# BoMingZhao/GaussianPrediction

Measured on AMD Instinct MI355X. Metric: rendered views/s (full train step) @1M Gaussians 1352x1014, higher is better.
Workload: dtype f32; 1 GPU; configs[2]: HyperNeRF-like 1M Gaussians, 1352x1014, stage-3 full train step (deform, raster, L1+SSIM loss, Adam: all HIP kernels); gaussians=1000000, width=1352, height=1014, keypoints=250, nearest_num=6, parallelism=view-parallel x1, ranks_seen_by_rccl=1, self_launched=False

## Files before the change

### gaussianprediction_amd/csrc/deform_kernels.hip

```cpp
#include "gp_common.h"
#include "deform_kernels.h"

typedef float f32x16 __attribute__((ext_vector_type(16)));

#define MLP_ROWS 32
#define MLP_THREADS 512
#define MLP_W 256

__device__ __forceinline__ int act_idx(int f, int j) { return f * MLP_ROWS + (j ^ (f & 31)); }
__device__ __forceinline__ int cd_row(int r, int half) { return (r & 3) + 8 * (r >> 2) + 4 * half; }

__device__ __forceinline__ void build_input(float* buf, const MlpDev& p, long row0, int tid) {
    const int fd = p.feature_dim, xf = p.xyz_freq, tf = p.time_freq;
    for (int e = tid; e < fd * MLP_ROWS; e += MLP_THREADS) {
        const int jj = e / fd, f = e - jj * fd;
        const long row = row0 + jj;
        buf[act_idx(f, jj)] = row < p.rows ? p.feature[row * fd + f] : 0.f;
    }
    for (int e = tid; e < 3 * xf * MLP_ROWS; e += MLP_THREADS) {
        const int jj = e % MLP_ROWS, cf = e / MLP_ROWS;
        const int c = cf / xf, fr = cf - c * xf;
        const long row = row0 + jj;
        float sv = 0.f, cv = 0.f;
        if (row < p.rows) {
// ... 685 lines not shown
}
__global__ __launch_bounds__(256) void gp_blend_fwd_kernel(BlendDev a, float* __restrict__ xyz_t, float* __restrict__ q_t) { blend_fwd_body<0>(a, xyz_t, q_t); }
__global__ __launch_bounds__(256) void gp_blend_fwd6_kernel(BlendDev a, float* __restrict__ xyz_t, float* __restrict__ q_t) { blend_fwd_body<6>(a, xyz_t, q_t); }
__global__ __launch_bounds__(256) void gp_blend_fwd8_kernel(BlendDev a, float* __restrict__ xyz_t, float* __restrict__ q_t) { blend_fwd_body<8>(a, xyz_t, q_t); }
__global__ __launch_bounds__(256) void gp_blend_fwd6_i16_kernel(BlendDev a, float* __restrict__ xyz_t, float* __restrict__ q_t) { blend_fwd_body<6, true>(a, xyz_t, q_t); }
__global__ __launch_bounds__(256) void gp_blend_fwd8_i16_kernel(BlendDev a, float* __restrict__ xyz_t, float* __restrict__ q_t) { blend_fwd_body<8, true>(a, xyz_t, q_t); }

__device__ __forceinline__ void normalize_bwd(const float* v, const float* g, float* dv) {
    const float n = norm4(v), inv = 1.f / n;
    const float y[4] = {v[0] * inv, v[1] * inv, v[2] * inv, v[3] * inv};
    const float dot = y[0] * g[0] + y[1] * g[1] + y[2] * g[2] + y[3] * g[3];
#pragma unroll
    for (int k = 0; k < 4; ++k) dv[k] = (g[k] - y[k] * dot) * inv;
}

#define BB_LONG 20
#define BB_LONG_CAP 320
template <int NN, bool I16 = false>
__device__ __forceinline__ void blend_bwd_body(BlendDev a, const float* __restrict__ g_xyz_t,
                                               const float* __restrict__ g_q_t, float* __restrict__ g_delta,
                                               float* __restrict__ g_raw_w, float* __restrict__ g_xyz,
                                               float* __restrict__ g_rot, float* __restrict__ partial, const unsigned bid,
                                               const unsigned nblk) {
    extern __shared__ float s_dyn[];
    const int od = a.out_dim;
    const int nn = NN > 0 ? NN : a.nn;
    const int K = (int)a.K;
    const int tid = threadIdx.x;
    float* s_acc = s_dyn;
    float* s_delta = s_acc + (nn > 0 ? K * 7 : 0);
    int* s_cnt = (int*)(s_delta + (nn > 0 ? K * od : 0));
    int* s_base = s_cnt + (nn > 0 ? K : 0);
    float* s_g = (float*)(s_base + (nn > 0 ? K + 1 : 0));
    float* s_inv = s_g + 256 * 7;
    float* s_w = s_inv + (nn > 0 ? K : 0);
    unsigned short* s_sorted = (unsigned short*)(s_w + 256 * 2 * nn);
    __shared__ int s_wsum[4];
    __shared__ int s_nlong, s_long[BB_LONG_CAP];
    if (nn > 0) {
        for (int e = tid; e < K * 7; e += 256) s_acc[e] = 0.f;
        for (int e = tid; e < K * od; e += 256) s_delta[e] = a.delta[e];
        if (a.norm_rotation) {
            __syncthreads();
            for (int kp = tid; kp < K; kp += 256) {
                float* dl = s_delta + kp * od;
                const float v[4] = {dl[3], dl[4], dl[5], dl[6]};
                const float inv = 1.f / norm4(v);
                s_inv[kp] = inv;
                dl[3] = v[0] * inv; dl[4] = v[1] * inv; dl[5] = v[2] * inv; dl[6] = v[3] * inv;
            }
        }
    }
    const long chunks = (a.N + 255) / 256;
    for (long c = bid; c < chunks; c += nblk) {
        const long i = c * 256 + tid;
        const bool live = i < a.N;
        if (nn > 0) {
            for (int e = tid; e < K; e += 256) s_cnt[e] = 0;
            if (tid == 0) s_nlong = 0;
            __syncthreads();
        }
        int kps[NN > 0 ? NN : GP_MAX_NN], rk[NN > 0 ? NN : GP_MAX_NN];
        if (live) {
            const float gx[3] = {g_xyz_t[3 * i], g_xyz_t[3 * i + 1], g_xyz_t[3 * i + 2]};
            const float gq[4] = {g_q_t[4 * i], g_q_t[4 * i + 1], g_q_t[4 * i + 2], g_q_t[4 * i + 3]};
            const float r[4] = {a.rot[4 * i], a.rot[4 * i + 1], a.rot[4 * i + 2], a.rot[4 * i + 3]};
            float wx[NN > 0 ? NN : GP_MAX_NN], wr[NN > 0 ? NN : GP_MAX_NN];
            float dq[4] = {0.f, 0.f, 0.f, 0.f};
            if (nn > 0) {
                if constexpr (NN > 0) {
                    float raw[2 * (NN > 0 ? NN : 1)];
                    load_row_nn<NN, I16>(a, i, raw, kps);
                    softmax_n(raw, NN, wx);
                    softmax_n(raw + NN, NN, wr);
                } else {
                    softmax_n(a.raw_w + i * 2 * nn, nn, wx);
                    softmax_n(a.raw_w + i * 2 * nn + nn, nn, wr);
                }
#pragma unroll
                for (int k = 0; k < nn; ++k) {
                    if (NN == 0) kps[k] = a.knn16 ? (int)a.knn16[i * nn + k] : (int)a.knn[i * nn + k];
                    const float* dl = s_delta + kps[k] * od;
                    const float v[4] = {dl[3], dl[4], dl[5], dl[6]};
                    dq[0] = fmaf(wr[k], v[0], dq[0]); dq[1] = fmaf(wr[k], v[1], dq[1]);
                    dq[2] = fmaf(wr[k], v[2], dq[2]); dq[3] = fmaf(wr[k], v[3], dq[3]);
                }
            } else {
                const float* dl = a.delta + i * od;
                dq[0] = dl[3]; dq[1] = dl[4]; dq[2] = dl[5]; dq[3] = dl[6];
                if (a.norm_rotation) { const float inv = 1.f / norm4(dq); dq[0] *= inv; dq[1] *= inv; dq[2] *= inv; dq[3] *= inv; }
            }
            const float invq = 1.f / norm4(dq);
            const float q[4] = {dq[0] * invq, dq[1] * invq, dq[2] * invq, dq[3] * invq};
            g_xyz[3 * i] = gx[0]; g_xyz[3 * i + 1] = gx[1]; g_xyz[3 * i + 2] = gx[2];
            float pq[4];
            quat_mul(q, r, pq);
            float gp[4];
            normalize_bwd(pq, gq, gp);
            const float gqn[4] = {gp[0] * r[0] + gp[1] * r[1] + gp[2] * r[2] + gp[3] * r[3],
                                  -gp[0] * r[1] + gp[1] * r[0] - gp[2] * r[3] + gp[3] * r[2],
                                  -gp[0] * r[2] + gp[1] * r[3] + gp[2] * r[0] - gp[3] * r[1],
                                  -gp[0] * r[3] - gp[1] * r[2] + gp[2] * r[1] + gp[3] * r[0]};
            g_rot[4 * i + 0] = gp[0] * q[0] + gp[1] * q[1] + gp[2] * q[2] + gp[3] * q[3];
            g_rot[4 * i + 1] = -gp[0] * q[1] + gp[1] * q[0] + gp[2] * q[3] - gp[3] * q[2];
            g_rot[4 * i + 2] = -gp[0] * q[2] - gp[1] * q[3] + gp[2] * q[0] + gp[3] * q[1];
            g_rot[4 * i + 3] = -gp[0] * q[3] + gp[1] * q[2] - gp[2] * q[1] + gp[3] * q[0];
            float gdq[4];
            normalize_bwd(dq, gqn, gdq);
            if (nn > 0) {
                float gwx[NN > 0 ? NN : GP_MAX_NN], gwr[NN > 0 ? NN : GP_MAX_NN];
                float sx = 0.f, sr = 0.f;
#pragma unroll
                for (int k = 0; k < nn; ++k) {
                    const float* dl = s_delta + kps[k] * od;
                    gwx[k] = dl[0] * gx[0] + dl[1] * gx[1] + dl[2] * gx[2];
                    const float vn[4] = {dl[3], dl[4], dl[5], dl[6]};
                    gwr[k] = vn[0] * gdq[0] + vn[1] * gdq[1] + vn[2] * gdq[2] + vn[3] * gdq[3];
                    sx += wx[k] * gwx[k];
                    sr += wr[k] * gwr[k];
                    s_w[k * 256 + tid] = wx[k];
                    s_w[(nn + k) * 256 + tid] = wr[k];
// ... 16 lines not shown
                }
                s_g[0 * 256 + tid] = gx[0]; s_g[1 * 256 + tid] = gx[1]; s_g[2 * 256 + tid] = gx[2];
                s_g[3 * 256 + tid] = gdq[0]; s_g[4 * 256 + tid] = gdq[1]; s_g[5 * 256 + tid] = gdq[2]; s_g[6 * 256 + tid] = gdq[3];
            } else {
                const float* dl = a.delta + i * od;
                float gv[4] = {gdq[0], gdq[1], gdq[2], gdq[3]};
                if (a.norm_rotation) { const float v[4] = {dl[3], dl[4], dl[5], dl[6]}; normalize_bwd(v, gdq, gv); }
                float* gd = g_delta + i * od;
                gd[0] = gx[0]; gd[1] = gx[1]; gd[2] = gx[2];
                gd[3] = gv[0]; gd[4] = gv[1]; gd[5] = gv[2]; gd[6] = gv[3];
                for (int k = 7; k < od; ++k) gd[k] = 0.f;
            }
        }
        if (nn > 0) {
            __syncthreads();
            {
                const int per = (K + 255) / 256;
                const int b0 = tid * per;
                int loc = 0;
                for (int e = 0; e < per; ++e) if (b0 + e < K) loc += s_cnt[b0 + e];
                int inc = loc;
                inc = gp_wave_scan_add(inc);
                if ((tid & 63) == 63) s_wsum[tid >> 6] = inc;
                __syncthreads();
                int woff = 0;
                for (int w = 0; w < (tid >> 6); ++w) woff += s_wsum[w];
                int run = woff + inc - loc;
                for (int e = 0; e < per; ++e) if (b0 + e < K) { s_base[b0 + e] = run; run += s_cnt[b0 + e]; }
                if (tid == 255) s_base[K] = run;
            }
            __syncthreads();
            if (live) {
#pragma unroll
                for (int k = 0; k < nn; ++k) s_sorted[s_base[kps[k]] + rk[k]] = (unsigned short)((k << 8) | tid);
            }
            __syncthreads();
            for (int kp = tid; kp < K; kp += 256) {
                float sacc[7] = {0.f, 0.f, 0.f, 0.f, 0.f, 0.f, 0.f};
                const int pe = s_base[kp + 1];
                if (pe - s_base[kp] > BB_LONG) { s_long[atomicAdd(&s_nlong, 1)] = kp; continue; }
                for (int pp = s_base[kp]; pp < pe; pp += 2) {
                    const int e0 = s_sorted[pp], e1 = pp + 1 < pe ? s_sorted[pp + 1] : -1;
                    const int t0 = e0 & 255, k0 = e0 >> 8, t1 = e1 & 255, k1 = (e1 >> 8) & 15;
                    const float wx0 = s_w[k0 * 256 + t0], wr0 = s_w[(nn + k0) * 256 + t0];
                    const float wx1 = e1 >= 0 ? s_w[k1 * 256 + t1] : 0.f, wr1 = e1 >= 0 ? s_w[(nn + k1) * 256 + t1] : 0.f;
                    float g0[7], g1[7];
#pragma unroll
                    for (int cc = 0; cc < 7; ++cc) { g0[cc] = s_g[cc * 256 + t0]; g1[cc] = s_g[cc * 256 + t1]; }
                    sacc[0] = fmaf(wx0, g0[0], sacc[0]); sacc[1] = fmaf(wx0, g0[1], sacc[1]); sacc[2] = fmaf(wx0, g0[2], sacc[2]);
                    sacc[3] = fmaf(wr0, g0[3], sacc[3]); sacc[4] = fmaf(wr0, g0[4], sacc[4]);
                    sacc[5] = fmaf(wr0, g0[5], sacc[5]); sacc[6] = fmaf(wr0, g0[6], sacc[6]);
// ... 60 lines not shown
__global__ __launch_bounds__(256) void gp_blend_bwd8_i16_kernel(BB_ARGS) { blend_bwd_body<8, true>(a, g_xyz_t, g_q_t, g_delta, g_raw_w, g_xyz, g_rot, partial, blockIdx.x, gridDim.x); }

template <int NN, bool I16>
__device__ __forceinline__ void blend_bwd_ride_body(const BlendRideDev& r, BB_ARGS) {
    const unsigned riders = r.fin_blocks + r.adam_chunks;
    if (blockIdx.x < riders) {
        if (blockIdx.x < r.fin_blocks) {
            extern __shared__ float s_dyn[];
            double* s_tot = (double*)(((uintptr_t)s_dyn + 7) & ~(uintptr_t)7);
            loss_finalize_body(r.fin, (float*)(s_tot + 8), s_tot);
        } else {
            adam_chunk_body<256>(r.t, blockIdx.x - r.fin_blocks, threadIdx.x, r.b1, r.b2, r.eps, r.zero_grad, r.skip_flag);
        }
        return;
    }
    blend_bwd_body<NN, I16>(a, g_xyz_t, g_q_t, g_delta, g_raw_w, g_xyz, g_rot, partial, blockIdx.x - riders, gridDim.x - riders);
}
__global__ __launch_bounds__(256) void gp_blend_bwd6_ride_kernel(BlendRideDev r, BB_ARGS) { blend_bwd_ride_body<6, false>(r, a, g_xyz_t, g_q_t, g_delta, g_raw_w, g_xyz, g_rot, partial); }
__global__ __launch_bounds__(256) void gp_blend_bwd8_ride_kernel(BlendRideDev r, BB_ARGS) { blend_bwd_ride_body<8, false>(r, a, g_xyz_t, g_q_t, g_delta, g_raw_w, g_xyz, g_rot, partial); }
__global__ __launch_bounds__(256) void gp_blend_bwd6_i16_ride_kernel(BlendRideDev r, BB_ARGS) { blend_bwd_ride_body<6, true>(r, a, g_xyz_t, g_q_t, g_delta, g_raw_w, g_xyz, g_rot, partial); }
__global__ __launch_bounds__(256) void gp_blend_bwd8_i16_ride_kernel(BlendRideDev r, BB_ARGS) { blend_bwd_ride_body<8, true>(r, a, g_xyz_t, g_q_t, g_delta, g_raw_w, g_xyz, g_rot, partial); }

__global__ __launch_bounds__(1024) void gp_blend_bwd_reduce_kernel(const float* __restrict__ partial, int nblocks, int KA,
                                                                  int od, float* __restrict__ g_delta) {
    __shared__ float s_r[16][64];
    const int lane = threadIdx.x & 63, wave = threadIdx.x >> 6;
    const int e = blockIdx.x * 64 + lane;
    float v0 = 0.f, v1 = 0.f, v2 = 0.f, v3 = 0.f;
    if (e < KA) {
        int b = wave;
        for (; b + 240 < nblocks; b += 256) {
// ... 68 lines not shown
```

### gaussianprediction_amd/csrc/gp_capi_deform.hip

```cpp
#include "gp_common.h"
#include "deform_kernels.h"
#include "loss_adam_kernels.h"
#include <stdlib.h>

static int make_mlp(const gp_mlp_params* p, const gp_mlp_input* x, MlpDev& m) {
    if (!p || !x) GP_FAIL("null mlp params/input");
    if (p->width != 256 || p->depth != 4) GP_FAIL("Deformable_Field: only d=4, w=256 is implemented (got d=%d w=%d)", p->depth, p->width);
    if (p->out_dim < 7 || p->out_dim > 8) GP_FAIL("out_dim must be 7 or 8 (got %d)", p->out_dim);
    if (x->feature_dim <= 0 || x->feature_dim % 4 || x->xyz_freq < 0 || x->xyz_freq > 16 || x->time_freq < 0 || x->time_freq > 16)
        GP_FAIL("bad input encoding dims");
    const int in_dim = x->feature_dim + 6 * x->xyz_freq + 2 * x->time_freq;
    if (in_dim != p->in_dim) GP_FAIL("in_dim %d != feature_dim + 6*xyz_freq + 2*time_freq = %d", p->in_dim, in_dim);
    if (in_dim % 4 || in_dim > 256) GP_FAIL("in_dim %d must be a multiple of 4 and <= 256", in_dim);
    if (x->rows < 0) GP_FAIL("negative rows");
    for (int l = 0; l < 5; ++l)
        if (!p->w[l] || !p->b[l]) GP_FAIL("null weight pointer (layer %d)", l);
    if (x->rows > 0 && (!x->feature || (x->xyz_freq > 0 && !x->xyz) || (x->time_freq > 0 && !x->t))) GP_FAIL("null input pointer");
    m.rows = x->rows; m.in_dim = in_dim; m.in_pad = (in_dim + 7) / 8 * 8; m.out_dim = p->out_dim;
    m.feature_dim = x->feature_dim; m.xyz_freq = x->xyz_freq; m.time_freq = x->time_freq;
    for (int l = 0; l < 5; ++l) { m.w[l] = p->w[l]; m.b[l] = p->b[l]; }
    m.feature = x->feature; m.xyz = x->xyz; m.t = x->t;
    m.pk = p->packed;
    if (m.pk && ((uintptr_t)m.pk & 15) != 0) GP_FAIL("gp_mlp_params.packed must be 16-byte aligned");
    if (p->scratch && ((uintptr_t)p->scratch & 15) != 0) GP_FAIL("gp_mlp_params.scratch must be 16-byte aligned");
// ... 226 lines not shown
extern "C" int gp_blend_forward(const gp_blend_args* a, float* xyz_t, float* q_t, gp_stream_t stream_) {
    BlendDev b;
    if (make_blend(a, b)) return 1;
    if (b.N == 0) return 0;
    if (!xyz_t || !q_t) GP_FAIL("null output");
    { GpProfScope _p("blend_fwd", (hipStream_t)stream_);
        const bool al = (((uintptr_t)b.raw_w | (uintptr_t)b.knn) & 15) == 0;
        const bool i16 = b.knn16 != nullptr;
        hipLaunchKernelGGL(b.nn == 6 && al ? (i16 ? gp_blend_fwd6_i16_kernel : gp_blend_fwd6_kernel)
                           : b.nn == 8 && al ? (i16 ? gp_blend_fwd8_i16_kernel : gp_blend_fwd8_kernel) : gp_blend_fwd_kernel,
                       dim3(gp_blocks((size_t)b.N, 256)), dim3(256), 0, (hipStream_t)stream_, b, xyz_t, q_t);
    GP_LAUNCH_CHECK(); }
    return 0;
}

int gp_blend_backward_impl(const gp_blend_args* a, const float* dL_dxyz_t, const float* dL_dq_t, float* dL_ddelta, float* dL_draw_w,
                           float* dL_dxyz, float* dL_drot, gp_alloc_fn alloc, void* alloc_ctx, gp_stream_t stream_, GpBlendRider* rider) {
    BlendDev b;
    if (make_blend(a, b)) return 1;
    if (b.N == 0) return 0;
    if (!dL_dxyz_t || !dL_dq_t || !dL_ddelta || !dL_dxyz || !dL_drot) GP_FAIL("null argument");
    const bool al = (((uintptr_t)b.raw_w | (uintptr_t)b.knn | (uintptr_t)dL_draw_w) & 15) == 0;
    const bool i16 = b.knn16 != nullptr;
    const bool ride = rider && (rider->fin_armed || rider->adam.armed) && al && (b.nn == 6 || b.nn == 8);
    const unsigned adam_chunks = ride && rider->adam.armed ? rider->adam.chunks : 0u;
    unsigned blocks = gp_blocks((size_t)b.N, 256);
    const unsigned cap = adam_chunks > 0 ? 768u : 1024u;
    if (b.nn > 0 && blocks > cap) blocks = cap;
    const size_t lds = b.nn > 0 ? ((size_t)b.K * (7 + b.out_dim + 3) + 1 + 256 * 7 + 256 * 2 * (size_t)b.nn) * 4 + 256 * (size_t)b.nn * 2 + 16 : 256 * 8 * 4;
    if (lds > 64 * 1024) GP_FAIL("keypoint blend backward: K = %ld, nn = %d needs %zu B of LDS (> 64 KiB)", (long)b.K, b.nn, lds);
    float* partial = nullptr;
    const int KA = (int)b.K * 7;
    if (b.nn > 0) {
        if (!alloc) GP_FAIL("null allocator");
        partial = (float*)alloc(alloc_ctx, GP_BUF_TEMP, gp_align_up((size_t)blocks * KA * sizeof(float), 256));
        if (!partial) GP_FAIL("allocator returned NULL for TEMP");
    }
    { GpProfScope _p("blend_bwd", (hipStream_t)stream_);
    if (ride) {
        BlendRideDev r;
        memset(&r, 0, sizeof(r));
        if (adam_chunks) {
            r.t = rider->adam.t; r.b1 = rider->adam.b1; r.b2 = rider->adam.b2; r.eps = rider->adam.eps; r.zero_grad = rider->adam.zero_grad;
            r.skip_flag = rider->adam.skip_flag; r.adam_chunks = adam_chunks;
        }
        if (rider->fin_armed) { r.fin = rider->fin; r.fin_blocks = 1; }
        rider->adam.armed = rider->fin_armed = false;
        hipLaunchKernelGGL(b.nn == 6 ? (i16 ? gp_blend_bwd6_i16_ride_kernel : gp_blend_bwd6_ride_kernel)
                                     : (i16 ? gp_blend_bwd8_i16_ride_kernel : gp_blend_bwd8_ride_kernel),
                           dim3(r.fin_blocks + r.adam_chunks + blocks), dim3(256), lds, (hipStream_t)stream_, r, b, dL_dxyz_t, dL_dq_t, dL_ddelta,
                           dL_draw_w, dL_dxyz, dL_drot, partial);
    } else {
        hipLaunchKernelGGL(b.nn == 6 && al ? (i16 ? gp_blend_bwd6_i16_kernel : gp_blend_bwd6_kernel)
                           : b.nn == 8 && al ? (i16 ? gp_blend_bwd8_i16_kernel : gp_blend_bwd8_kernel) : gp_blend_bwd_kernel,
                           dim3(blocks), dim3(256), lds, (hipStream_t)stream_, b, dL_dxyz_t, dL_dq_t, dL_ddelta,
                           dL_draw_w, dL_dxyz, dL_drot, partial);
    }
    GP_LAUNCH_CHECK();
    if (b.nn > 0) {
        hipLaunchKernelGGL(gp_blend_bwd_reduce_kernel, dim3(gp_blocks((size_t)KA, 64)), dim3(1024), 0, (hipStream_t)stream_, partial,
                           (int)blocks, KA, b.out_dim, dL_ddelta);
        GP_LAUNCH_CHECK();
// ... 33 lines not shown
```

### gaussianprediction_amd/csrc/gp_train_step.hip

```cpp
#include "gp_common.h"
#include "loss_adam_kernels.h"

__global__ __launch_bounds__(256) void gp_step_accumulate_kernel(float* __restrict__ dst, const float* __restrict__ src, int64_t n) {
    const int64_t i = (int64_t)blockIdx.x * 256 + threadIdx.x;
    if (i < n) dst[i] += src[i];
}

static int step_adam(const gp_step_update* u, uint32_t sel, gp_stream_t stream, GpAdamRider* ride = nullptr) {
    float *P[32], *G[32], *M[32], *V[32];
    int64_t NUM[32], ST[32];
    float LR[32];
    int n = 0;
    uint32_t keep = 0;
    for (int k = 0; k < u->adam_count && k < 32; ++k) {
        if (!((sel >> k) & 1u)) continue;
        P[n] = u->adam_params[k]; G[n] = u->adam_grads[k]; M[n] = u->adam_exp_avgs[k]; V[n] = u->adam_exp_avg_sqs[k];
        NUM[n] = u->adam_numels[k]; LR[n] = u->adam_lrs[k];
        ST[n] = u->adam_steps ? u->adam_steps[k] : u->step;
        if ((u->keep_grad_mask >> k) & 1u) keep |= 1u << n;
        ++n;
    }
    if (n == 0) return 0;
    if (ride) return gp_adam_rider_fill(ride, n, P, G, M, V, NUM, LR, ST, u->beta1, u->beta2, u->eps, 1, keep, u->skip_flag);
    return gp_adam_step_multi_steps(n, P, G, M, V, NUM, LR, ST, u->beta1, u->beta2, u->eps, 1, keep, u->skip_flag, stream);
}

static int train_step_run(const gp_step_plan* p, const gp_step_view* v, const gp_step_update* u, gp_alloc_fn alloc, void* alloc_ctx,
                          gp_stream_t stream, bool& temp_open);
extern "C" int gp_train_step_run(const gp_step_plan* p, const gp_step_view* v, const gp_step_update* u, gp_alloc_fn alloc,
                                 void* alloc_ctx, gp_stream_t stream) {
    bool temp_open = false;
    const int rc = train_step_run(p, v, u, alloc, alloc_ctx, stream, temp_open);
    if (rc && temp_open) alloc(alloc_ctx, GP_BUF_TEMP_DONE, 0);
    return rc;
}
static int train_step_run(const gp_step_plan* p, const gp_step_view* v, const gp_step_update* u, gp_alloc_fn alloc, void* alloc_ctx,
                          gp_stream_t stream, bool& temp_open) {
    if (!p || !v || !u || !alloc) GP_FAIL("gp_train_step_run: null argument");
    const int64_t N = p->num_gaussians, K = p->num_keypoints;
    if (N <= 0 || K <= 0 || p->nearest_num <= 0) GP_FAIL("gp_train_step_run: needs Gaussians, keypoints and neighbours (the stage-3 form)");
    if (u->binning_capacity <= 0 || !u->binning_status) GP_FAIL("gp_train_step_run: capacity mode only (binning_capacity > 0 with a status word)");
// ... 39 lines not shown
    in.opacities = raw_act ? p->opacity : p->opacity_t;
    in.scales = raw_act ? p->scaling : p->scale; in.rotations = p->q_t;
    gp_raster_outputs out = p->out;
    gp_raster_saved saved;
    memset(&saved, 0, sizeof(saved));
    if (gp_raster_forward(&st, &in, &out, &saved, alloc, alloc_ctx, stream)) return 1;
    alloc(alloc_ctx, GP_BUF_TEMP_DONE, 0);
    if (u->hook) u->hook(u->hook_ctx, GP_STEP_AFTER_FORWARD);

    float* dimg = p->dL_dimage;
    if (!dimg) GP_FAIL("gp_train_step_run: null intermediate buffer");
    const int riders_off = gp_debug_get(15);
    GpLossPrologue pro;
    pro.armed = false;
    GpBlendRider blend_riders;
    blend_riders.fin_armed = blend_riders.adam.armed = false;
    if (gp_debug_get(11) == 0) {
        if (!(riders_off & 1)) {
            if (gp_raster_backward_prepare(&st, &in, &saved, alloc, alloc_ctx, &pro)) return 1;
            temp_open = pro.armed;
        }
        if (gp_loss_l1_ssim_fused_impl(out.color, v->gt_image, 3, H, W, p->lambda_dssim, nullptr, p->loss_sums, dimg, reg ? p->keypoint_features : nullptr,
                                       nfeat, p->reg_scale, reg ? p->g_keypoint_features : nullptr, stream, &pro)) return 1;
        if (!(riders_off & 2)) {
            if (gp_loss_finalize_fill(&blend_riders.fin, p->loss_sums, 3, H, W, p->lambda_dssim, reg ? p->keypoint_features : nullptr, nfeat,
                                      p->reg_scale, p->loss)) return 1;
            blend_riders.fin_armed = true;
        } else if (reg) { if (gp_loss_l1_ssim_finalize_reg(p->loss_sums, 3, H, W, p->lambda_dssim, p->keypoint_features, nfeat, p->reg_scale, p->loss, stream)) return 1; }
        else if (gp_loss_l1_ssim_finalize(p->loss_sums, 3, H, W, p->lambda_dssim, p->loss, stream)) return 1;
    } else {
        float* dmaps = p->dmaps;
// ... 3 lines not shown
        }
        if (gp_loss_l1_ssim_forward(out.color, v->gt_image, 3, H, W, p->loss_sums, dmaps, stream)) return 1;
        if (reg) {
            if (gp_loss_l1_ssim_finalize_reg(p->loss_sums, 3, H, W, p->lambda_dssim, p->keypoint_features, nfeat, p->reg_scale, p->loss, stream)) return 1;
            if (gp_loss_l1_ssim_backward_reg(out.color, v->gt_image, dmaps, 3, H, W, p->lambda_dssim, nullptr, dimg,
                                             p->keypoint_features, nfeat, p->reg_scale, p->g_keypoint_features, stream)) return 1;
        } else {
            if (gp_loss_l1_ssim_finalize(p->loss_sums, 3, H, W, p->lambda_dssim, p->loss, stream)) return 1;
            if (gp_loss_l1_ssim_backward(out.color, v->gt_image, dmaps, 3, H, W, p->lambda_dssim, nullptr, dimg, stream)) return 1;
        }
        if (!p->dmaps) alloc(alloc_ctx, GP_BUF_TEMP_DONE, 0);
    }

    gp_raster_grads g;
    memset(&g, 0, sizeof(g));
    g.dL_dmeans3D = p->g_xyz_t; g.dL_dmeans2D = p->g_means2D; g.dL_dshs = p->g_features_dc; g.dL_dshs_rest = p->g_features_rest;
    g.dL_dopacities = raw_act ? p->g_opacity : p->g_opacity_t; g.dL_dscales = raw_act ? p->g_scaling : p->g_scale; g.dL_drotations = p->g_q_t; g.accumulate_shs = 0; g.adam_shs = u->adam_shs;
    if (gp_raster_backward_impl(&st, &in, &out, &saved, dimg, nullptr, &g, alloc, alloc_ctx, stream, pro.armed ? pro.acc : nullptr)) return 1;
    alloc(alloc_ctx, GP_BUF_TEMP_DONE, 0);
    temp_open = false;
    if (u->hook) u->hook(u->hook_ctx, GP_STEP_AFTER_RASTER_BACKWARD);
    if (!raw_act && gp_activations_backward(N, p->scaling, p->opacity, nullptr, 0, 1.f, p->g_scale, p->g_opacity_t, p->g_scaling, p->g_opacity, nullptr, stream))
        return 1;
    const uint32_t all = u->adam_count >= 32 ? 0xFFFFFFFFu : ((1u << u->adam_count) - 1u);
    uint32_t rode = 0;
    if (!(riders_off & 4) && raw_act && !u->hook)
        for (int k = 0; k < u->adam_count; ++k)
            if (u->adam_params[k] == p->scaling || u->adam_params[k] == p->opacity) rode |= 1u << k;
    if (rode && step_adam(u, rode, stream, &blend_riders.adam)) return 1;
    if (gp_blend_backward_impl(&ba, p->g_xyz_t, p->g_q_t, p->g_delta, nullptr, p->g_xyz, p->g_rotation, alloc, alloc_ctx, stream, &blend_riders)) return 1;
    alloc(alloc_ctx, GP_BUF_TEMP_DONE, 0);
    if (blend_riders.fin_armed && gp_loss_finalize_launch(blend_riders.fin, (hipStream_t)stream)) return 1;
    if (gp_adam_rider_launch(&blend_riders.adam, (hipStream_t)stream)) return 1;
    const uint32_t early = (u->hook || u->adam_count <= 0) ? 0u : (u->adam_early_mask & all & ~rode);
    GpAdamRider mlp_rider;
    mlp_rider.armed = false;
    if (early && step_adam(u, early, stream, &mlp_rider)) return 1;
    gp_mlp_grads mg = p->g_mlp;
    const bool add_in_place = reg && gp_mlp_backward_splits(&p->mlp, K);
    if (gp_mlp_backward_impl(&p->mlp, &mi, p->acts, p->g_delta, &mg, (reg && !add_in_place) ? p->g_feature_tmp : p->g_keypoint_features,
                             p->g_keypoints, alloc, alloc_ctx, stream, &mlp_rider, add_in_place)) return 1;
    if (gp_adam_rider_launch(&mlp_rider, (hipStream_t)stream)) return 1;
    if (reg && !add_in_place) {
        hipLaunchKernelGGL(gp_step_accumulate_kernel, dim3(gp_blocks((size_t)nfeat, 256)), dim3(256), 0, (hipStream_t)stream,
                           p->g_keypoint_features, (const float*)p->g_feature_tmp, nfeat);
        GP_LAUNCH_CHECK();
    }
    if (u->hook) u->hook(u->hook_ctx, GP_STEP_AFTER_BACKWARD);

    if (u->adam_count > 0 && step_adam(u, all & ~early & ~rode, stream)) return 1;
    return 0;
}
```

### gaussianprediction_amd/csrc/loss_adam_kernels.h

```cpp
#pragma once
#include "gp_common.h"

#define ADAM_MAX_TENSORS 32
#define ADAM_CHUNK 16384
struct AdamTable {
    float* p[ADAM_MAX_TENSORS];
    float* g[ADAM_MAX_TENSORS];
    float* m[ADAM_MAX_TENSORS];
    float* v[ADAM_MAX_TENSORS];
    unsigned long long n[ADAM_MAX_TENSORS];
    float step_size[ADAM_MAX_TENSORS];
    float bc2_sqrt[ADAM_MAX_TENSORS];
    unsigned keep_grad_mask;
    unsigned chunk_begin[ADAM_MAX_TENSORS + 1];
    int count;
};

template <int THREADS>
__device__ __forceinline__ void adam_chunk_body(const AdamTable& t, unsigned chunk, int tid, float b1, float b2, float eps, int zero_grad,
                                                const uint32_t* __restrict__ skip_flag) {
    const bool skip = skip_flag && *skip_flag != 0;
    int k = 0;
    while (k + 1 < t.count && chunk >= t.chunk_begin[k + 1]) ++k;
    const size_t base = (size_t)(chunk - t.chunk_begin[k]) * ADAM_CHUNK;
    const size_t n = t.n[k];
    float* __restrict__ p = t.p[k]; float* __restrict__ g = t.g[k]; float* __restrict__ m = t.m[k]; float* __restrict__ v = t.v[k];
    const float step_size = t.step_size[k], bc2_sqrt = t.bc2_sqrt[k];
    if ((t.keep_grad_mask >> k) & 1u) zero_grad = 0;
    const size_t end = base + ADAM_CHUNK < n ? base + ADAM_CHUNK : n;
    auto upd = [&](float4& pv, const float4& gv, float4& mv, float4& vv) {
        float* pp = (float*)&pv; const float* gg = (const float*)&gv; float* mm = (float*)&mv; float* vq = (float*)&vv;
#pragma unroll
        for (int u = 0; u < 4; ++u) gp_adam_update(pp[u], gg[u], mm[u], vq[u], b1, b2, eps, step_size, bc2_sqrt);
    };
    const float4 zero4 = make_float4(0.f, 0.f, 0.f, 0.f);
    size_t i = base + (size_t)tid * 4;
    if (skip) {
        if (zero_grad)
            for (size_t j = base + tid; j < end; j += THREADS) g[j] = 0.f;
        return;
    }
    constexpr size_t S = (size_t)THREADS * 4;
    for (; i + S + 3 < end; i += 2 * S) {
        const size_t j = i + S;
// ... 98 lines not shown
        }
        tot = block_sum_256(acc, s_red);
    }
    double s0, s1;
    loss_slot_totals(f.sums, f.nslots, s_tot, s0, s1);
    if (threadIdx.x == 0) {
        const float l = (float)((1.0 - (double)f.lambda) * s0 / f.n + (double)f.lambda * (1.0 - s1 / f.n));
        f.loss[0] = f.x ? l + tot * f.scale_over_n : l;
    }
}

int gp_loss_finalize_fill(LossFinalizeDev* f, const double* sums, int32_t channels, int32_t H, int32_t W, float lambda_dssim, const float* x,
                          int64_t n, float scale, float* loss);
int gp_loss_finalize_launch(const LossFinalizeDev& f, hipStream_t s);

struct BlendRideDev {
    AdamTable t;
    float b1, b2, eps;
    int zero_grad;
    const uint32_t* skip_flag;
    unsigned adam_chunks;
    unsigned fin_blocks;
    LossFinalizeDev fin;
};
struct GpBlendRider {
    GpAdamRider adam;
    LossFinalizeDev fin;
    bool fin_armed;
};
int gp_blend_backward_impl(const gp_blend_args* a, const float* dL_dxyz_t, const float* dL_dq_t, float* dL_ddelta, float* dL_draw_w,
                           float* dL_dxyz, float* dL_drot, gp_alloc_fn alloc, void* alloc_ctx, gp_stream_t stream, GpBlendRider* riders);

struct GpLossPrologue {
    const int2* ranges;
    const int32_t* tile_work;
    int T;
    uint32_t* order;
    float* acc;
    size_t acc_floats;
    bool armed;
};
int gp_raster_backward_prepare(const gp_raster_settings* st, const gp_raster_inputs* in, const gp_raster_saved* saved, gp_alloc_fn alloc,
                               void* alloc_ctx, GpLossPrologue* pro);
int gp_loss_l1_ssim_fused_impl(const float* img, const float* gt, int32_t channels, int32_t H, int32_t W, float lambda_dssim,
// ... 6 lines not shown
```

### gaussianprediction_amd/csrc/loss_adam_kernels.hip

```cpp
#include "gp_common.h"
#include "loss_adam_kernels.h"
#include "raster_kernels.h"

#define GP_LOSS_REG_MAX 65536
#define LT 32
#define LH 5
#define LE (LT + 2 * LH)
#define LP (LE + 1)
#define LHP (LT + 1)

struct Win11 { float w[11]; };

__global__ __launch_bounds__(256) void gp_l1_ssim_fwd_kernel(const float* __restrict__ img, const float* __restrict__ gt,
                                                            int H, int W, Win11 win, double* __restrict__ sums,
                                                            float* __restrict__ dmap) {
    __shared__ float s_a[LE][LP], s_b[LE][LP];
    __shared__ float s_h[4][LE][LHP];
    __shared__ float s_red[4];
    const int tid = threadIdx.x;
    const int tx0 = blockIdx.x * LT, ty0 = blockIdx.y * LT, ch = blockIdx.z;
    const size_t HW = (size_t)H * W;
    const float* a_img = img + ch * HW;
    const float* b_img = gt + ch * HW;
    {
// ... 542 lines not shown
                       (size_t)n, lr, beta1, beta2, eps, bc1, bc2_sqrt, zero_grad);
    GP_LAUNCH_CHECK();
    return 0;
}

static int adam_build_table(AdamTable& t, long& n_chunks, int32_t count, float* const* params, float* const* grads, float* const* exp_avgs,
                            float* const* exp_avg_sqs, const int64_t* numels, const float* lrs, const int64_t* steps, float beta1,
                            float beta2, uint32_t keep_grad_mask) {
    n_chunks = 0;
    if (count < 0 || count > ADAM_MAX_TENSORS) GP_FAIL("adam: at most %d tensors per call (got %d)", ADAM_MAX_TENSORS, count);
    if (count == 0) return 0;
    if (!params || !grads || !exp_avgs || !exp_avg_sqs || !numels || !lrs || !steps) GP_FAIL("null argument");
    t.count = 0;
    t.keep_grad_mask = 0;
    unsigned chunks = 0;
    for (int k = 0; k < count; ++k) {
        if (numels[k] <= 0) continue;
        if (steps[k] < 1) GP_FAIL("adam: bad step %lld (tensor %d)", (long long)steps[k], k);
        if ((((uintptr_t)params[k] | (uintptr_t)grads[k] | (uintptr_t)exp_avgs[k] | (uintptr_t)exp_avg_sqs[k]) & 15) != 0)
            GP_FAIL("adam: pointers must be 16-byte aligned (tensor %d)", k);
        const int j = t.count++;
        if ((keep_grad_mask >> k) & 1u) t.keep_grad_mask |= 1u << j;
        t.p[j] = params[k]; t.g[j] = grads[k]; t.m[j] = exp_avgs[k]; t.v[j] = exp_avg_sqs[k];
        t.n[j] = (unsigned long long)numels[k];
        t.step_size[j] = lrs[k] / (1.f - powf(beta1, (float)steps[k]));
        t.bc2_sqrt[j] = sqrtf(1.f - powf(beta2, (float)steps[k]));
        t.chunk_begin[j] = chunks;
        chunks += (unsigned)((numels[k] + ADAM_CHUNK - 1) / ADAM_CHUNK);
    }
    t.chunk_begin[t.count] = chunks;
    n_chunks = (long)chunks;
    return 0;
}

int gp_adam_rider_fill(GpAdamRider* r, int count, float* const* params, float* const* grads, float* const* exp_avgs,
                       float* const* exp_avg_sqs, const int64_t* numels, const float* lrs, const int64_t* steps, float beta1, float beta2,
                       float eps, int zero_grad, uint32_t keep_grad_mask, const uint32_t* skip_flag) {
    r->armed = false;
    long chunks = 0;
    if (adam_build_table(r->t, chunks, count, params, grads, exp_avgs, exp_avg_sqs, numels, lrs, steps, beta1, beta2, keep_grad_mask)) return 1;
    r->b1 = beta1; r->b2 = beta2; r->eps = eps; r->zero_grad = zero_grad; r->skip_flag = skip_flag; r->chunks = (unsigned)chunks;
    r->armed = chunks > 0;
    return 0;
// ... 54 lines not shown
```

Measured before the change: 870.6 views/s.

## Fuse Adam updates for xyz, rotation, scaling, opacity into blend backward kernel

Moves the Adam optimizer updates for the per-Gaussian xyz, rotation, scaling and opacity tensors into the blend backward kernel, applying them as each gradient is produced. This removes separate Adam passes that re-read gradients, params and moments, and lets xyz gradients skip a copy from g_xyz_t. It also adds a smaller Adam chunk size for small launches so they spread over more blocks. The cost is more register and memory pressure inside the blend backward kernel and a more complex ordering of writes around barriers.

```diff
diff --git a/gaussianprediction_amd/csrc/deform_kernels.hip b/gaussianprediction_amd/csrc/deform_kernels.hip
--- a/gaussianprediction_amd/csrc/deform_kernels.hip
+++ b/gaussianprediction_amd/csrc/deform_kernels.hip
@@ -723,14 +723,43 @@
     for (int k = 0; k < 4; ++k) dv[k] = (g[k] - y[k] * dot) * inv;
 }
 
+struct OwnSpan { float4 p, g, m, v; };
+__device__ __forceinline__ void own_span_load(OwnSpan& o, const float* p, const float* g, const float* m, const float* v, long off) {
+    o.p = *(const float4*)(p + off); o.g = *(const float4*)(g + off); o.m = *(const float4*)(m + off); o.v = *(const float4*)(v + off);
+}
+__device__ __forceinline__ void own_span_step(OwnSpan& o, float* p, float* zero, float* m, float* v, long off, bool skip, float b1, float b2,
+                                              float eps, float step_size, float bc2_sqrt) {
+    if (!skip) {
+        float* pp = (float*)&o.p; const float* gg = (const float*)&o.g; float* mm = (float*)&o.m; float* vv = (float*)&o.v;
+#pragma unroll
+        for (int u = 0; u < 4; ++u) gp_adam_update(pp[u], gg[u], mm[u], vv[u], b1, b2, eps, step_size, bc2_sqrt);
+        *(float4*)(p + off) = o.p; *(float4*)(m + off) = o.m; *(float4*)(v + off) = o.v;
+    }
+    if (zero) *(float4*)(zero + off) = make_float4(0.f, 0.f, 0.f, 0.f);
+}
+template <int W>
+__device__ __forceinline__ void own_row_step(float* p, const float* g, float* zero, float* m, float* v, long row, bool skip, float b1, float b2,
+                                             float eps, float step_size, float bc2_sqrt) {
+    for (int k = 0; k < W; ++k) {
+        const long e = row * W + k;
+        if (!skip) {
+            float pe = p[e], me = m[e], ve = v[e];
+            gp_adam_update(pe, g[e], me, ve, b1, b2, eps, step_size, bc2_sqrt);
+            p[e] = pe; m[e] = me; v[e] = ve;
+        }
+        if (zero) zero[e] = 0.f;
+    }
+}
+
 #define BB_LONG 20
 #define BB_LONG_CAP 320
-template <int NN, bool I16 = false>
+template <int NN, bool I16 = false, bool OWN = false>
 __device__ __forceinline__ void blend_bwd_body(BlendDev a, const float* __restrict__ g_xyz_t,
                                                const float* __restrict__ g_q_t, float* __restrict__ g_delta,
                                                float* __restrict__ g_raw_w, float* __restrict__ g_xyz,
                                                float* __restrict__ g_rot, float* __restrict__ partial, const unsigned bid,
-                                               const unsigned nblk) {
+                                               const unsigned nblk,
+                                               const BlendOwnAdamDev* own_ = nullptr) {
     extern __shared__ float s_dyn[];
     const int od = a.out_dim;
     const int nn = NN > 0 ? NN : a.nn;
@@ -760,6 +789,15 @@
             }
         }
     }
+    bool ox = false, orot = false, os = false, oo = false, own_skip = false;
+    if constexpr (OWN) {
+        if (own_->on) {
+            ox = own_->s[BLEND_OWN_XYZ].present != 0; orot = own_->s[BLEND_OWN_ROT].present != 0;
+            os = own_->s[BLEND_OWN_SCALING].present != 0; oo = own_->s[BLEND_OWN_OPACITY].present != 0;
+            own_skip = own_->skip_flag && *own_->skip_flag != 0;
+        }
+    }
+    const bool copy_xyz = g_xyz != g_xyz_t;
     const long chunks = (a.N + 255) / 256;
     for (long c = bid; c < chunks; c += nblk) {
         const long i = c * 256 + tid;
@@ -774,6 +812,17 @@
             const float gx[3] = {g_xyz_t[3 * i], g_xyz_t[3 * i + 1], g_xyz_t[3 * i + 2]};
             const float gq[4] = {g_q_t[4 * i], g_q_t[4 * i + 1], g_q_t[4 * i + 2], g_q_t[4 * i + 3]};
             const float r[4] = {a.rot[4 * i], a.rot[4 * i + 1], a.rot[4 * i + 2], a.rot[4 * i + 3]};
+            float rm[4] = {0.f, 0.f, 0.f, 0.f}, rv[4] = {0.f, 0.f, 0.f, 0.f};
+            auto load_rot_moments = [&]() {
+                if constexpr (OWN) {
+                    if (orot && !own_skip) {
+                        const BlendOwnAdamSlot& t = own_->s[BLEND_OWN_ROT];
+#pragma unroll
+                        for (int k = 0; k < 4; ++k) { rm[k] = t.m[4 * i + k]; rv[k] = t.v[4 * i + k]; }
+                    }
+                }
+            };
+            load_rot_moments();
             float wx[NN > 0 ? NN : GP_MAX_NN], wr[NN > 0 ? NN : GP_MAX_NN];
             float dq[4] = {0.f, 0.f, 0.f, 0.f};
             if (nn > 0) {
@@ -801,7 +850,10 @@
             }
             const float invq = 1.f / norm4(dq);
             const float q[4] = {dq[0] * invq, dq[1] * invq, dq[2] * invq, dq[3] * invq};
-            g_xyz[3 * i] = gx[0]; g_xyz[3 * i + 1] = gx[1]; g_xyz[3 * i + 2] = gx[2];
+            if (copy_xyz) {
+                const bool z = ox && own_->s[BLEND_OWN_XYZ].zero_g;
+                g_xyz[3 * i] = z ? 0.f : gx[0]; g_xyz[3 * i + 1] = z ? 0.f : gx[1]; g_xyz[3 * i + 2] = z ? 0.f : gx[2];
+            }
             float pq[4];
             quat_mul(q, r, pq);
             float gp[4];
@@ -810,10 +862,26 @@
                                   -gp[0] * r[1] + gp[1] * r[0] - gp[2] * r[3] + gp[3] * r[2],
                                   -gp[0] * r[2] + gp[1] * r[3] + gp[2] * r[0] - gp[3] * r[1],
                                   -gp[0] * r[3] - gp[1] * r[2] + gp[2] * r[1] + gp[3] * r[0]};
-            g_rot[4 * i + 0] = gp[0] * q[0] + gp[1] * q[1] + gp[2] * q[2] + gp[3] * q[3];
-            g_rot[4 * i + 1] = -gp[0] * q[1] + gp[1] * q[0] + gp[2] * q[3] - gp[3] * q[2];
-            g_rot[4 * i + 2] = -gp[0] * q[2] - gp[1] * q[3] + gp[2] * q[0] + gp[3] * q[1];
-            g_rot[4 * i + 3] = -gp[0] * q[3] + gp[1] * q[2] - gp[2] * q[1] + gp[3] * q[0];
+            const float gr[4] = {gp[0] * q[0] + gp[1] * q[1] + gp[2] * q[2] + gp[3] * q[3],
+                                 -gp[0] * q[1] + gp[1] * q[0] + gp[2] * q[3] - gp[3] * q[2],
+                                 -gp[0] * q[2] - gp[1] * q[3] + gp[2] * q[0] + gp[3] * q[1],
+                                 -gp[0] * q[3] + gp[1] * q[2] - gp[2] * q[1] + gp[3] * q[0]};
+            {
+                const bool z = orot && own_->s[BLEND_OWN_ROT].zero_g;
+#pragma unroll
+                for (int k = 0; k < 4; ++k) g_rot[4 * i + k] = z ? 0.f : gr[k];
+            }
+            if constexpr (OWN) {
+                if (orot && !own_skip) {
+                    const BlendOwnAdamSlot& t = own_->s[BLEND_OWN_ROT];
+                    float rp[4] = {r[0], r[1], r[2], r[3]};
+#pragma unroll
+                    for (int k = 0; k < 4; ++k) {
+                        gp_adam_update(rp[k], gr[k], rm[k], rv[k], own_->b1, own_->b2, own_->eps, t.step_size, t.bc2_sqrt);
+                        t.p[4 * i + k] = rp[k]; t.m[4 * i + k] = rm[k]; t.v[4 * i + k] = rv[k];
+                    }
+                }
+            }
             float gdq[4];
             normalize_bwd(dq, gqn, gdq);
             if (nn > 0) {
@@ -860,6 +928,24 @@
         }
         if (nn > 0) {
             __syncthreads();
+            const float4 zero4 = make_float4(0.f, 0.f, 0.f, 0.f);
+            OwnSpan sx = {zero4, zero4, zero4, zero4}, so = sx;
+            const long wrow = c * 256 + (tid & ~63);
+            const int wrows = a.N - wrow >= 64 ? 64 : (a.N - wrow > 0 ? (int)(a.N - wrow) : 0);
+            const bool wfull = wrows == 64;
+            const int f0 = 4 * (tid & 63);
+            if constexpr (OWN) {
+                if (!own_skip && wfull) {
+                    if (ox && f0 < 3 * 64) {
+                        const BlendOwnAdamSlot& t = own_->s[BLEND_OWN_XYZ];
+                        own_span_load(sx, t.p, g_xyz_t, t.m, t.v, wrow * 3 + f0);
+                    }
+                    if (oo && f0 < 64) {
+                        const BlendOwnAdamSlot& t = own_->s[BLEND_OWN_OPACITY];
+                        own_span_load(so, t.p, t.g, t.m, t.v, wrow + f0);
+                    }
+                }
+            }
             {
                 const int per = (K + 255) / 256;
                 const int b0 = tid * per;
@@ -876,11 +962,43 @@
                 if (tid == 255) s_base[K] = run;
             }
             __syncthreads();
+            OwnSpan ss = {zero4, zero4, zero4, zero4};
+            if constexpr (OWN) {
+                if (own_->on) {
+                    const float b1 = own_->b1, b2 = own_->b2, eps = own_->eps;
+                    if (ox && !own_skip) {
+                        const BlendOwnAdamSlot& t = own_->s[BLEND_OWN_XYZ];
+                        if (wfull) { if (f0 < 3 * 64) own_span_step(sx, t.p, nullptr, t.m, t.v, wrow * 3 + f0, false, b1, b2, eps, t.step_size, t.bc2_sqrt); }
+                        else if (live) own_row_step<3>(t.p, g_xyz_t, nullptr, t.m, t.v, i, false, b1, b2, eps, t.step_size, t.bc2_sqrt);
+                    }
+                    if (oo) {
+                        const BlendOwnAdamSlot& t = own_->s[BLEND_OWN_OPACITY];
+                        float* const zero = t.zero_g ? t.g : nullptr;
+                        if (wfull) { if (f0 < 64) own_span_step(so, t.p, zero, t.m, t.v, wrow + f0, own_skip, b1, b2, eps, t.step_size, t.bc2_sqrt); }
+                        else if (live) own_row_step<1>(t.p, t.g, zero, t.m, t.v, i, own_skip, b1, b2, eps, t.step_size, t.bc2_sqrt);
+                    }
+                    if (os && !own_skip && wfull && f0 < 3 * 64) {
+                        const BlendOwnAdamSlot& t = own_->s[BLEND_OWN_SCALING];
+                        own_span_load(ss, t.p, t.g, t.m, t.v, wrow * 3 + f0);
+                    }
+                }
+            }
             if (live) {
 #pragma unroll
                 for (int k = 0; k < nn; ++k) s_sorted[s_base[kps[k]] + rk[k]] = (unsigned short)((k << 8) | tid);
             }
             __syncthreads();
+            if constexpr (OWN) {
+                if (own_->on) {
+                    const float b1 = own_->b1, b2 = own_->b2, eps = own_->eps;
+                    if (os) {
+                        const BlendOwnAdamSlot& t = own_->s[BLEND_OWN_SCALING];
+                        float* const zero = t.zero_g ? t.g : nullptr;
+                        if (wfull) { if (f0 < 3 * 64) own_span_step(ss, t.p, zero, t.m, t.v, wrow * 3 + f0, own_skip, b1, b2, eps, t.step_size, t.bc2_sqrt); }
+                        else if (live) own_row_step<3>(t.p, t.g, zero, t.m, t.v, i, own_skip, b1, b2, eps, t.step_size, t.bc2_sqrt);
+                    }
+                }
+            }
             for (int kp = tid; kp < K; kp += 256) {
                 float sacc[7] = {0.f, 0.f, 0.f, 0.f, 0.f, 0.f, 0.f};
                 const int pe = s_base[kp + 1];
@@ -971,7 +1089,7 @@
         }
         return;
     }
-    blend_bwd_body<NN, I16>(a, g_xyz_t, g_q_t, g_delta, g_raw_w, g_xyz, g_rot, partial, blockIdx.x - riders, gridDim.x - riders);
+    blend_bwd_body<NN, I16, NN == 6>(a, g_xyz_t, g_q_t, g_delta, g_raw_w, g_xyz, g_rot, partial, blockIdx.x - riders, gridDim.x - riders, &r.own);
 }
 __global__ __launch_bounds__(256) void gp_blend_bwd6_ride_kernel(BlendRideDev r, BB_ARGS) { blend_bwd_ride_body<6, false>(r, a, g_xyz_t, g_q_t, g_delta, g_raw_w, g_xyz, g_rot, partial); }
 __global__ __launch_bounds__(256) void gp_blend_bwd8_ride_kernel(BlendRideDev r, BB_ARGS) { blend_bwd_ride_body<8, false>(r, a, g_xyz_t, g_q_t, g_delta, g_raw_w, g_xyz, g_rot, partial); }
diff --git a/gaussianprediction_amd/csrc/gp_capi_deform.hip b/gaussianprediction_amd/csrc/gp_capi_deform.hip
--- a/gaussianprediction_amd/csrc/gp_capi_deform.hip
+++ b/gaussianprediction_amd/csrc/gp_capi_deform.hip
@@ -264,6 +264,10 @@
     return 0;
 }
 
+bool gp_blend_backward_applies_adam(const gp_blend_args* a) {
+    return a && a->nearest_num == 6 && (((uintptr_t)a->raw_w | (uintptr_t)a->knn_idx) & 15) == 0;
+}
+
 int gp_blend_backward_impl(const gp_blend_args* a, const float* dL_dxyz_t, const float* dL_dq_t, float* dL_ddelta, float* dL_draw_w,
                            float* dL_dxyz, float* dL_drot, gp_alloc_fn alloc, void* alloc_ctx, gp_stream_t stream_, GpBlendRider* rider) {
     BlendDev b;
@@ -272,7 +276,8 @@
     if (!dL_dxyz_t || !dL_dq_t || !dL_ddelta || !dL_dxyz || !dL_drot) GP_FAIL("null argument");
     const bool al = (((uintptr_t)b.raw_w | (uintptr_t)b.knn | (uintptr_t)dL_draw_w) & 15) == 0;
     const bool i16 = b.knn16 != nullptr;
-    const bool ride = rider && (rider->fin_armed || rider->adam.armed) && al && (b.nn == 6 || b.nn == 8);
+    const bool ride = rider && (rider->fin_armed || rider->adam.armed || rider->own_armed) && al && (b.nn == 6 || b.nn == 8);
+    const bool own = ride && rider->own_armed && b.nn == 6;
     const unsigned adam_chunks = ride && rider->adam.armed ? rider->adam.chunks : 0u;
     unsigned blocks = gp_blocks((size_t)b.N, 256);
     const unsigned cap = adam_chunks > 0 ? 768u : 1024u;
@@ -286,7 +291,7 @@
         partial = (float*)alloc(alloc_ctx, GP_BUF_TEMP, gp_align_up((size_t)blocks * KA * sizeof(float), 256));
         if (!partial) GP_FAIL("allocator returned NULL for TEMP");
     }
-    { GpProfScope _p("blend_bwd", (hipStream_t)stream_);
+    { GpProfScope _p(own ? "adam" : "blend_bwd", (hipStream_t)stream_);
     if (ride) {
         BlendRideDev r;
         memset(&r, 0, sizeof(r));
@@ -295,7 +300,9 @@
             r.skip_flag = rider->adam.skip_flag; r.adam_chunks = adam_chunks;
         }
         if (rider->fin_armed) { r.fin = rider->fin; r.fin_blocks = 1; }
+        if (own) r.own = rider->own;
         rider->adam.armed = rider->fin_armed = false;
+        if (own) rider->own_armed = false;
         hipLaunchKernelGGL(b.nn == 6 ? (i16 ? gp_blend_bwd6_i16_ride_kernel : gp_blend_bwd6_ride_kernel)
                                      : (i16 ? gp_blend_bwd8_i16_ride_kernel : gp_blend_bwd8_ride_kernel),
                            dim3(r.fin_blocks + r.adam_chunks + blocks), dim3(256), lds, (hipStream_t)stream_, r, b, dL_dxyz_t, dL_dq_t, dL_ddelta,
diff --git a/gaussianprediction_amd/csrc/gp_train_step.hip b/gaussianprediction_amd/csrc/gp_train_step.hip
--- a/gaussianprediction_amd/csrc/gp_train_step.hip
+++ b/gaussianprediction_amd/csrc/gp_train_step.hip
@@ -25,6 +25,39 @@
     return gp_adam_step_multi_steps(n, P, G, M, V, NUM, LR, ST, u->beta1, u->beta2, u->eps, 1, keep, u->skip_flag, stream);
 }
 
+
+static int step_own_adam(const gp_step_plan* p, const gp_step_update* u, bool raw_act, BlendOwnAdamDev* own, uint32_t* taken) {
+    memset(own, 0, sizeof(*own));
+    *taken = 0;
+    const int64_t N = p->num_gaussians;
+    const float* const P[4] = {p->xyz, p->rotation, p->scaling, p->opacity};
+    float* const G[4] = {p->g_xyz, p->g_rotation, p->g_scaling, p->g_opacity};
+    const int64_t NUM[4] = {3 * N, 4 * N, 3 * N, N};
+    int slot_of[32];
+    uint32_t sel = 0;
+    for (int k = 0; k < u->adam_count && k < 32; ++k)
+        for (int s = 0; s < 4; ++s) {
+            if (s >= BLEND_OWN_SCALING && !raw_act) continue;
+            if (u->adam_params[k] == P[s] && u->adam_grads[k] == G[s] && u->adam_numels[k] == NUM[s] && !own->s[s].present) {
+                own->s[s].present = 1; slot_of[k] = s; sel |= 1u << k;
+            }
+        }
+    if (!sel) return 0;
+    GpAdamRider r;
+    if (step_adam(u, sel, nullptr, &r)) return 1;
+    int j = 0;
+    for (int k = 0; k < u->adam_count && k < 32; ++k) {
+        if (!((sel >> k) & 1u)) continue;
+        BlendOwnAdamSlot& t = own->s[slot_of[k]];
+        t.p = r.t.p[j]; t.g = r.t.g[j]; t.m = r.t.m[j]; t.v = r.t.v[j];
+        t.step_size = r.t.step_size[j]; t.bc2_sqrt = r.t.bc2_sqrt[j];
+        t.zero_g = r.zero_grad && !((r.t.keep_grad_mask >> j) & 1u);
+        ++j;
+    }
+    own->b1 = r.b1; own->b2 = r.b2; own->eps = r.eps; own->skip_flag = r.skip_flag; own->on = 1;
+    *taken = sel;
+    return 0;
+}
 static int train_step_run(const gp_step_plan* p, const gp_step_view* v, const gp_step_update* u, gp_alloc_fn alloc, void* alloc_ctx,
                           gp_stream_t stream, bool& temp_open);
 extern "C" int gp_train_step_run(const gp_step_plan* p, const gp_step_view* v, const gp_step_update* u, gp_alloc_fn alloc,
@@ -94,7 +127,7 @@
     GpLossPrologue pro;
     pro.armed = false;
     GpBlendRider blend_riders;
-    blend_riders.fin_armed = blend_riders.adam.armed = false;
+    blend_riders.fin_armed = blend_riders.adam.armed = blend_riders.own_armed = false;
     if (gp_debug_get(11) == 0) {
         if (!(riders_off & 1)) {
             if (gp_raster_backward_prepare(&st, &in, &saved, alloc, alloc_ctx, &pro)) return 1;
@@ -128,7 +161,15 @@
 
     gp_raster_grads g;
     memset(&g, 0, sizeof(g));
-    g.dL_dmeans3D = p->g_xyz_t; g.dL_dmeans2D = p->g_means2D; g.dL_dshs = p->g_features_dc; g.dL_dshs_rest = p->g_features_rest;
+    const uint32_t all = u->adam_count >= 32 ? 0xFFFFFFFFu : ((1u << u->adam_count) - 1u);
+    uint32_t own = 0;
+    if (!(riders_off & 8) && !u->hook && u->adam_count > 0 && gp_blend_backward_applies_adam(&ba)) {
+        if (step_own_adam(p, u, raw_act, &blend_riders.own, &own)) return 1;
+        blend_riders.own_armed = own != 0;
+    }
+    const BlendOwnAdamSlot& own_xyz = blend_riders.own.s[BLEND_OWN_XYZ];
+    float* const g_xyz_t = (blend_riders.own_armed && own_xyz.present && !own_xyz.zero_g) ? p->g_xyz : p->g_xyz_t;
+    g.dL_dmeans3D = g_xyz_t; g.dL_dmeans2D = p->g_means2D; g.dL_dshs = p->g_features_dc; g.dL_dshs_rest = p->g_features_rest;
     g.dL_dopacities = raw_act ? p->g_opacity : p->g_opacity_t; g.dL_dscales = raw_act ? p->g_scaling : p->g_scale; g.dL_drotations = p->g_q_t; g.accumulate_shs = 0; g.adam_shs = u->adam_shs;
     if (gp_raster_backward_impl(&st, &in, &out, &saved, dimg, nullptr, &g, alloc, alloc_ctx, stream, pro.armed ? pro.acc : nullptr)) return 1;
     alloc(alloc_ctx, GP_BUF_TEMP_DONE, 0);
@@ -136,17 +177,17 @@
     if (u->hook) u->hook(u->hook_ctx, GP_STEP_AFTER_RASTER_BACKWARD);
     if (!raw_act && gp_activations_backward(N, p->scaling, p->opacity, nullptr, 0, 1.f, p->g_scale, p->g_opacity_t, p->g_scaling, p->g_opacity, nullptr, stream))
         return 1;
-    const uint32_t all = u->adam_count >= 32 ? 0xFFFFFFFFu : ((1u << u->adam_count) - 1u);
     uint32_t rode = 0;
     if (!(riders_off & 4) && raw_act && !u->hook)
         for (int k = 0; k < u->adam_count; ++k)
-            if (u->adam_params[k] == p->scaling || u->adam_params[k] == p->opacity) rode |= 1u << k;
+            if ((u->adam_params[k] == p->scaling || u->adam_params[k] == p->opacity) && !((own >> k) & 1u)) rode |= 1u << k;
     if (rode && step_adam(u, rode, stream, &blend_riders.adam)) return 1;
-    if (gp_blend_backward_impl(&ba, p->g_xyz_t, p->g_q_t, p->g_delta, nullptr, p->g_xyz, p->g_rotation, alloc, alloc_ctx, stream, &blend_riders)) return 1;
+    if (gp_blend_backward_impl(&ba, g_xyz_t, p->g_q_t, p->g_delta, nullptr, p->g_xyz, p->g_rotation, alloc, alloc_ctx, stream, &blend_riders)) return 1;
     alloc(alloc_ctx, GP_BUF_TEMP_DONE, 0);
+    if (blend_riders.own_armed) GP_FAIL("gp_train_step_run: the blend backward did not apply the optimizer update planned for it");
     if (blend_riders.fin_armed && gp_loss_finalize_launch(blend_riders.fin, (hipStream_t)stream)) return 1;
     if (gp_adam_rider_launch(&blend_riders.adam, (hipStream_t)stream)) return 1;
-    const uint32_t early = (u->hook || u->adam_count <= 0) ? 0u : (u->adam_early_mask & all & ~rode);
+    const uint32_t early = (u->hook || u->adam_count <= 0) ? 0u : (u->adam_early_mask & all & ~rode & ~own);
     GpAdamRider mlp_rider;
     mlp_rider.armed = false;
     if (early && step_adam(u, early, stream, &mlp_rider)) return 1;
@@ -162,6 +203,6 @@
     }
     if (u->hook) u->hook(u->hook_ctx, GP_STEP_AFTER_BACKWARD);
 
-    if (u->adam_count > 0 && step_adam(u, all & ~early & ~rode, stream)) return 1;
+    if (u->adam_count > 0 && step_adam(u, all & ~early & ~rode & ~own, stream)) return 1;
     return 0;
 }
diff --git a/gaussianprediction_amd/csrc/loss_adam_kernels.h b/gaussianprediction_amd/csrc/loss_adam_kernels.h
--- a/gaussianprediction_amd/csrc/loss_adam_kernels.h
+++ b/gaussianprediction_amd/csrc/loss_adam_kernels.h
@@ -3,6 +3,8 @@
 
 #define ADAM_MAX_TENSORS 32
 #define ADAM_CHUNK 16384
+#define ADAM_CHUNK_SMALL 2048
+#define ADAM_SMALL_LAUNCH (1 << 20)
 struct AdamTable {
     float* p[ADAM_MAX_TENSORS];
     float* g[ADAM_MAX_TENSORS];
@@ -13,6 +15,7 @@
     float bc2_sqrt[ADAM_MAX_TENSORS];
     unsigned keep_grad_mask;
     unsigned chunk_begin[ADAM_MAX_TENSORS + 1];
+    unsigned chunk;
     int count;
 };
 
@@ -22,12 +25,12 @@
     const bool skip = skip_flag && *skip_flag != 0;
     int k = 0;
     while (k + 1 < t.count && chunk >= t.chunk_begin[k + 1]) ++k;
-    const size_t base = (size_t)(chunk - t.chunk_begin[k]) * ADAM_CHUNK;
+    const size_t base = (size_t)(chunk - t.chunk_begin[k]) * t.chunk;
     const size_t n = t.n[k];
     float* __restrict__ p = t.p[k]; float* __restrict__ g = t.g[k]; float* __restrict__ m = t.m[k]; float* __restrict__ v = t.v[k];
     const float step_size = t.step_size[k], bc2_sqrt = t.bc2_sqrt[k];
     if ((t.keep_grad_mask >> k) & 1u) zero_grad = 0;
-    const size_t end = base + ADAM_CHUNK < n ? base + ADAM_CHUNK : n;
+    const size_t end = base + t.chunk < n ? base + t.chunk : n;
     auto upd = [&](float4& pv, const float4& gv, float4& mv, float4& vv) {
         float* pp = (float*)&pv; const float* gg = (const float*)&gv; float* mm = (float*)&mv; float* vq = (float*)&vv;
 #pragma unroll
@@ -156,8 +159,22 @@
                           int64_t n, float scale, float* loss);
 int gp_loss_finalize_launch(const LossFinalizeDev& f, hipStream_t s);
 
+struct BlendOwnAdamSlot {
+    float* p; float* g; float* m; float* v;
+    float step_size, bc2_sqrt;
+    int present;
+    int zero_g;
+};
+enum { BLEND_OWN_XYZ = 0, BLEND_OWN_ROT = 1, BLEND_OWN_SCALING = 2, BLEND_OWN_OPACITY = 3 };
+struct BlendOwnAdamDev {
+    BlendOwnAdamSlot s[4];
+    float b1, b2, eps;
+    const uint32_t* skip_flag;
+    int on;
+};
 struct BlendRideDev {
     AdamTable t;
+    BlendOwnAdamDev own;
     float b1, b2, eps;
     int zero_grad;
     const uint32_t* skip_flag;
@@ -169,7 +186,10 @@
     GpAdamRider adam;
     LossFinalizeDev fin;
     bool fin_armed;
-};
+    BlendOwnAdamDev own;
+    bool own_armed;
+};
+bool gp_blend_backward_applies_adam(const gp_blend_args* a);
 int gp_blend_backward_impl(const gp_blend_args* a, const float* dL_dxyz_t, const float* dL_dq_t, float* dL_ddelta, float* dL_draw_w,
                            float* dL_dxyz, float* dL_drot, gp_alloc_fn alloc, void* alloc_ctx, gp_stream_t stream, GpBlendRider* riders);
 
diff --git a/gaussianprediction_amd/csrc/loss_adam_kernels.hip b/gaussianprediction_amd/csrc/loss_adam_kernels.hip
--- a/gaussianprediction_amd/csrc/loss_adam_kernels.hip
+++ b/gaussianprediction_amd/csrc/loss_adam_kernels.hip
@@ -580,6 +580,9 @@
     t.count = 0;
     t.keep_grad_mask = 0;
     unsigned chunks = 0;
+    int64_t total = 0;
+    for (int k = 0; k < count; ++k) total += numels[k] > 0 ? numels[k] : 0;
+    t.chunk = total <= ADAM_SMALL_LAUNCH ? ADAM_CHUNK_SMALL : ADAM_CHUNK;
     for (int k = 0; k < count; ++k) {
         if (numels[k] <= 0) continue;
         if (steps[k] < 1) GP_FAIL("adam: bad step %lld (tensor %d)", (long long)steps[k], k);
@@ -592,7 +595,7 @@
         t.step_size[j] = lrs[k] / (1.f - powf(beta1, (float)steps[k]));
         t.bc2_sqrt[j] = sqrtf(1.f - powf(beta2, (float)steps[k]));
         t.chunk_begin[j] = chunks;
-        chunks += (unsigned)((numels[k] + ADAM_CHUNK - 1) / ADAM_CHUNK);
+        chunks += (unsigned)((numels[k] + t.chunk - 1) / t.chunk);
     }
     t.chunk_begin[t.count] = chunks;
     n_chunks = (long)chunks;
```

Result: no change. 872.4 views/s (median of 6 runs) (+0.2%).
